# arnavdantuluri/StableTriton

Hardware: AMD Instinct MI355X
Metric: denoise it/s, SDXL UNet 1024x1024 50-step, bs=1 per GPU (higher is better)
Workload: dtype bf16; 1 GPU; SDXL-base UNet, latent 128x128 (1024x1024 px), bs=1/GPU, 50-step Euler-discrete loop, hipGraph mode=step, no CFG; parallelism=prompt-parallel x1, weights=synthetic seed 0, weight_broadcasts=0

## Files before the change

stabletriton_amd/csrc/dispatch.h:

```cpp
#pragma once
#include "gemm_reg.h"
#include "gemm_dma.h"
#include "gemm8p.h"
#ifdef ST_DEV_CONFIGS
#include "../../tools/dev_kernels/gemm4w.h"
void gemm4w_bf16(const GemmArgs& a, hipStream_t st);
void gemm4w_f16(const GemmArgs& a, hipStream_t st);
void gemm4w_fp8(const GemmArgs& a, hipStream_t st);
template <typename T> static inline void gemm4w_call(const GemmArgs& a, hipStream_t st) {
    if constexpr (std::is_same<T, bf16>::value) gemm4w_bf16(a, st);
    else if constexpr (std::is_same<T, f16>::value) gemm4w_f16(a, st);
    else gemm4w_fp8(a, st);
}
#endif

static inline bool colstats_ok(const GemmArgs& a, int bm, bool lnf) {
    const bool ok = a.col_stats && !lnf && (a.N & 3) == 0 && a.rows_per_batch > 0 && a.rows_per_batch % bm == 0 &&
                    cdiv(a.M, bm) <= a.col_tiles_cap;
    if (a.col_rows_out) *a.col_rows_out = ok ? bm : 0;
    return ok;
}

template <typename T, int BM, int BN, int WGM, int WGN, int STAGES, int U, bool CONV, bool GEGLU, bool LNF, bool XA = false>
static void launch_dma_one(const GemmArgs& a, hipStream_t st, int tiles_n) {
    const size_t lds = (size_t)STAGES * U * (BM + BN) * 128 + (size_t)BM * 8 + 1024;
    const int sk = a.splitk > 1 ? a.splitk : 1;
    auto kfn = gemm_dma_kernel<T, BM, BN, WGM, WGN, STAGES, U, CONV, GEGLU, LNF, XA>;
    const bool emit_cols = colstats_ok(a, BM, LNF);
    static unsigned long long lds_ok = 0;
    ensure_dynamic_lds(kfn, lds, &lds_ok);
    GemmArgs b = a;
    {
        static const int force_pm = dev_env_int("ST_GEMM_PANELS", 0);
        const int tiles_m = cdiv(a.M, BM);
        const double abytes = CONV ? (double)a.M * a.Cin * (a.ups ? 0.25 : 1.0) * a.stride * a.stride : (double)a.M * a.K;
        const double wbytes = (double)(GEGLU ? 2 : 1) * a.N * a.K;
        int best_p = 1;
        double best = 1e300;
        for (int pm = 1; pm <= 8; pm *= 2) {
            if (pm > tiles_m) break;
            const double c = abytes * (8.0 / pm) + wbytes * pm;
            if (c < best) { best = c; best_p = pm; }
        }
        if (force_pm > 0) best_p = force_pm > tiles_m ? tiles_m : force_pm;
        b.panel_h = cdiv(tiles_m, best_p);
    }
    const int main_blocks = cdiv(a.M, BM) * tiles_n * sk;
    b.splitk = sk;
    fill_tile_map(b, cdiv(a.M, BM), tiles_n, a.K / ((128 / (int)sizeof(T)) * U));
    static const bool no_helpers = dev_env_int("ST_NO_HELPER_BLOCKS", 0) != 0;
    b.helper_blocks = (b.next_w && main_blocks <= 208 && !no_helpers) ? (256 - main_blocks > 96 ? 96 : 256 - main_blocks) : 0;
    if (!emit_cols) b.col_stats = nullptr;
    fill_next_per(b, main_blocks + b.helper_blocks);
    hipLaunchKernelGGL(kfn, dim3(main_blocks + b.helper_blocks), dim3(WGM * WGN * 64), lds, st, b);
}

template <typename T, int BM, int BN, int WGM, int WGN, int STAGES, int U, bool CONV>
static void launch_dma(const GemmArgs& a, hipStream_t st) {
    if constexpr (!CONV) {
        const bool geglu = a.epi & ST_EPI_GEGLU;
        constexpr bool PAIRS = (BN % 32 == 0);
        if (a.ln_c) {
            if constexpr (PAIRS) {
                if (geglu) { launch_dma_one<T, BM, BN, WGM, WGN, STAGES, U, false, true, true>(a, st, cdiv(a.N, BN / 2)); return; }
            }
            launch_dma_one<T, BM, BN, WGM, WGN, STAGES, U, false, false, true>(a, st, cdiv(a.N, BN));
            return;
        }
        if constexpr (PAIRS) {
            if (geglu) { launch_dma_one<T, BM, BN, WGM, WGN, STAGES, U, false, true, false>(a, st, cdiv(a.N, BN / 2)); return; }
        }
    }
    launch_dma_one<T, BM, BN, WGM, WGN, STAGES, U, CONV, false, false>(a, st, cdiv(a.N, BN));
}

enum { CFG_64x64_S4 = 0, CFG_64x64_S8 = 1, CFG_64x64_S4_U2 = 2, CFG_128x64_S4 = 3, CFG_128x64_S3_U2 = 4,
       CFG_128x128_S3 = 5, CFG_64x64_S3 = 6, CFG_64x64_W8 = 7, CFG_128x64_W8 = 8, CFG_128x128_W8 = 9,
       CFG_64x128_W8 = 10, CFG_64x128_W8_S6 = 11, CFG_128x64_W8_S6 = 12, CFG_128x128_W8_S4 = 13, CFG_64x64_W8_S8 = 14, CFG_64x128_W8_U2 = 15, CFG_128x64_W8_U2 = 16, CFG_64x64_W8_U2 = 17, CFG_256x256_W8 = 18, CFG_256x128_W8 = 19, CFG_128x128_W8_S2 = 20, CFG_128x64_W8_S3 = 21, CFG_64x128_W8_S3 = 22, CFG_128x320_W8 = 23, CFG_128x256_W8 = 24, CFG_64x320_W8 = 25, CFG_64x80_W4 = 26, CFG_128x80_W8 = 27, CFG_128x160_W8 = 28, CFG_128x128_N4_S2 = 29, CFG_128x64_N4_S3 = 30, CFG_64x128_N4_S3 = 31, CFG_256x160_W8_S2 = 32, CFG_COUNT, CFG_256x256_8P = 100, CFG_256x160_8P = 101, CFG_256x256_4W = 102 };

static inline int cfg_bn(int cfg) {
    switch (cfg) {
        case CFG_64x64_S4: case CFG_64x64_S8: case CFG_64x64_S4_U2: case CFG_128x64_S4: case CFG_128x64_S3_U2: case CFG_64x64_S3:
        case CFG_64x64_W8: case CFG_128x64_W8: case CFG_128x64_W8_S6: case CFG_64x64_W8_S8: case CFG_128x64_W8_U2:
        case CFG_64x64_W8_U2: case CFG_128x64_W8_S3: case CFG_128x64_N4_S3: return 64;
        case CFG_256x256_W8: case CFG_128x256_W8: return 256;
        case CFG_128x320_W8: case CFG_64x320_W8: return 320;
        case CFG_64x80_W4: case CFG_128x80_W8: return 80;
        case CFG_128x160_W8: case CFG_256x160_W8_S2: return 160;
        default: return 128;
    }
}

#ifdef ST_DEV_CONFIGS
extern int g_dbg_cfg, g_dbg_fusek;
#endif
static inline int forced_cfg() {
    static int v = dev_env_int("ST_GEMM_FORCE", -1);
#ifdef ST_DEV_CONFIGS
    if (g_dbg_cfg >= 0) return g_dbg_cfg;
#endif
    return v;
}

#ifndef ST_TW_128x128
#define ST_TW_128x128 1.0
#endif
#ifndef ST_TW_64x128
#define ST_TW_64x128 1.0
#endif
#ifndef ST_TW_128x64
#define ST_TW_128x64 1.0
#endif
#ifndef ST_TW_64x64
#define ST_TW_64x64 1.0
#endif
#ifndef ST_TW_128x80
#define ST_TW_128x80 1.0
#endif
#ifndef ST_TW_128x160
#define ST_TW_128x160 1.0
#endif
#ifndef ST_TW_SPLITK
#define ST_TW_SPLITK 1.0
#endif
#ifndef ST_TW_8P
#define ST_TW_8P 1.1
#endif
static inline double model_tweak(int cfg) {
    switch (cfg) {
        case 9: return ST_TW_128x128;
        case 10: return ST_TW_64x128;
        case 8: return ST_TW_128x64;
        case 7: return ST_TW_64x64;
        case 27: return ST_TW_128x80;
        case 28: return ST_TW_128x160;
        default: return 1.0;
    }
}
#ifndef ST_SPLIT_DENSE_TRIP
#define ST_SPLIT_DENSE_TRIP 1.0
#endif
#ifndef ST_SPLIT_160_TRIP
#define ST_SPLIT_160_TRIP 0.8
#endif
// ... 207 lines not shown
```

stabletriton_amd/csrc/epilogue.h:

```cpp
#pragma once
#include "gemm_args.h"

template <typename T, bool GEGLU>
__device__ __forceinline__ void epilogue_compute4(const GemmArgs& p, int m, int n, float (&v)[4], const float (&g_in)[4],
                                                  float ln_mean = 0.f, float ln_rstd = 0.f) {
    const T* __restrict__ bias = (const T*)p.bias;
    const T* __restrict__ Rp = (const T*)p.residual;
    const T* __restrict__ RBp = (const T*)p.rowbias;
    const bool full = (n + 3 < p.N);
    float g[4];
#pragma unroll
    for (int e = 0; e < 4; ++e) g[e] = g_in[e];
    if (p.col_scale) {
        const float rs = p.row_scale[(size_t)m * p.rs_stride];
        for (int e = 0; e < 4 && n + e < p.N; ++e) { v[e] *= rs * p.col_scale[n + e]; if (GEGLU) g[e] *= rs * p.col_scale[p.Ng + n + e]; }
    }
    if (p.ln_c) {
        if (full) {
            float c4[4], d4[4];
            Out4<float>::load(p.ln_c + n, c4); Out4<float>::load(p.ln_d + n, d4);
#pragma unroll
            for (int e = 0; e < 4; ++e) v[e] = ln_fold(v[e], ln_mean, ln_rstd, c4[e], d4[e]);
            if (GEGLU) {
                Out4<float>::load(p.ln_c + p.Ng + n, c4); Out4<float>::load(p.ln_d + p.Ng + n, d4);
// ... 549 lines not shown
    }
    if (has_q8) publish_amax(p.q8_amax, q8_max, blockIdx.x * (NT / 64) + (threadIdx.x >> 6));
    retire_touches(touch_next);
}

template <typename TO, int BM, int BN, int WGM, int WGN, int TM, int TN, bool GEGLU, int LDS_BYTES, bool STATS, bool SCALED = false, typename ColMap>
__device__ __forceinline__ void staged_epilogue(const GemmArgs& p, f32x4 (&acc)[TM][TN], int m0, int n0, int tile_n, int wm, int r16, int q,
                                                ColMap colmap, char* lds, const float2* lnrows) {
    constexpr int VEC = EpiVec<TO>::N;
    constexpr int BNO = GEGLU ? BN / 2 : BN;
    const bool has_res = p.epi & ST_EPI_RESIDUAL, has_rb = p.epi & ST_EPI_ROWBIAS;
    const bool aligned = (m0 + BM <= p.M) && (n0 + BNO <= p.N) && (p.N % VEC == 0) &&
                         (p.C == nullptr || ((p.ldc % VEC == 0) && ((uintptr_t)p.C & 15) == 0)) &&
                         (!has_res || ((p.ldr % VEC == 0) && ((uintptr_t)p.residual & 15) == 0)) && (!has_rb || ((uintptr_t)p.rowbias & 15) == 0) &&
                         ((((uintptr_t)p.bias | (uintptr_t)p.ln_c | (uintptr_t)p.ln_d | (uintptr_t)p.col_scale) & 15) == 0) &&
                         (p.q8_out == nullptr || VEC == 8);
    if (aligned) {
        const int flags = ((p.epi & ST_EPI_BIAS) ? EPI_F_BIAS : 0) | (has_res ? EPI_F_RES : 0) | (has_rb ? EPI_F_RB : 0) | (p.ln_c ? EPI_F_LN : 0) |
                          ((p.epi & ST_EPI_SILU) ? EPI_F_SILU : 0) | (p.col_scale ? EPI_F_SCALE : 0) | ((STATS && p.row_stats) ? EPI_F_ROWS : 0) |
                          ((STATS && p.col_stats && (p.N & 3) == 0) ? EPI_F_COLS : 0) | (p.q8_out ? EPI_F_Q8 : 0) | (p.C ? 0 : EPI_F_NOC) |
                          (p.sp_out ? EPI_F_SP : 0);
#define ST_EPI_CASE(M)                                                                                                                          \
    case (M):                                                                                                                                   \
        staged_epilogue_impl<TO, BM, BN, WGM, WGN, TM, TN, GEGLU, LDS_BYTES, STATS, (M)>(p, acc, m0, n0, tile_n, wm, r16, q, colmap, lds, lnrows); \
        return;
        if constexpr (std::is_same<TO, float>::value) {
            if constexpr (!STATS && !SCALED) {
                switch (flags) { ST_EPI_CASE(EPI_F_LN | EPI_F_SP) default: break; }
            } else if constexpr (STATS && !SCALED) {
                switch (flags) {
                    ST_EPI_CASE(EPI_F_BIAS | EPI_F_ROWS | EPI_F_SP)
                    ST_EPI_CASE(EPI_F_BIAS | EPI_F_RES | EPI_F_ROWS | EPI_F_SP)
                    default: break;
                }
            }
        }
        if constexpr (!STATS && !SCALED) {
            switch (flags) { ST_EPI_CASE(EPI_F_LN) ST_EPI_CASE(EPI_F_LN | EPI_F_BIAS) default: break; }
        } else if constexpr (!STATS && SCALED) {
            switch (flags) {
                ST_EPI_CASE(EPI_F_LN | EPI_F_SCALE)
                ST_EPI_CASE(EPI_F_LN | EPI_F_SCALE | EPI_F_Q8 | EPI_F_NOC)
                default: break;
            }
        } else if constexpr (STATS && !SCALED) {
            switch (flags) {
                ST_EPI_CASE(EPI_F_BIAS)
                ST_EPI_CASE(EPI_F_BIAS | EPI_F_RES)
                ST_EPI_CASE(EPI_F_BIAS | EPI_F_ROWS)
                ST_EPI_CASE(EPI_F_BIAS | EPI_F_RES | EPI_F_ROWS)
                ST_EPI_CASE(EPI_F_BIAS | EPI_F_RES | EPI_F_ROWS | EPI_F_Q8)
                ST_EPI_CASE(EPI_F_BIAS | EPI_F_COLS)
                ST_EPI_CASE(EPI_F_BIAS | EPI_F_RB | EPI_F_COLS)
                ST_EPI_CASE(EPI_F_BIAS | EPI_F_RES | EPI_F_COLS)
                default: break;
            }
        } else {
            switch (flags) {
                ST_EPI_CASE(EPI_F_BIAS | EPI_F_SCALE | EPI_F_RES | EPI_F_ROWS)
                ST_EPI_CASE(EPI_F_BIAS | EPI_F_SCALE | EPI_F_RES | EPI_F_ROWS | EPI_F_Q8)
                default: break;
            }
        }
#undef ST_EPI_CASE
    }
    staged_epilogue_impl<TO, BM, BN, WGM, WGN, TM, TN, GEGLU, LDS_BYTES, STATS, -1>(p, acc, m0, n0, tile_n, wm, r16, q, colmap, lds, lnrows);
}

typedef __attribute__((address_space(3))) void epi_lds_void_t;
typedef __attribute__((address_space(1))) const void epi_gbl_cvoid_t;
__device__ __forceinline__ void touch_next_weights_dma(const GemmArgs& p, unsigned lds_dump_addr) {
    if (!p.next_w || p.helper_blocks > 0) return;
    const size_t lines = p.next_bytes >> 7;
    const size_t per = p.next_per ? (size_t)p.next_per : (lines + gridDim.x - 1) / gridDim.x;
    const size_t lo = (size_t)blockIdx.x * per, hi = lo + per < lines ? lo + per : lines;
    const size_t step = blockDim.x;
    for (size_t l = lo + threadIdx.x; l < hi; l += step)
        __builtin_amdgcn_global_load_lds((epi_gbl_cvoid_t*)((const char*)p.next_w + (touch_line(p, l) << 7)), (epi_lds_void_t*)(uintptr_t)lds_dump_addr, 4, 0, 0);
}

struct DirectCol { int col; bool gate; };
template <int TN, bool GEGLU>
__host__ __device__ __forceinline__ constexpr DirectCol direct_col(int j, int rho) {
    static_assert(TN == 4 || TN == 5, "direct epilogue: wave tiles of 64 or 80 columns");
    const int pc = 8 * (rho >> 2) + (rho & 3);
    if (TN == 4) {
        if (GEGLU) return DirectCol{pc + 4 * (j & 1), j >= 2};
        return DirectCol{32 * (j >> 1) + pc + 4 * (j & 1), false};
    }
    if (GEGLU) {
        if (j < 2) return DirectCol{pc + 4 * j, false};
        if (j > 2) return DirectCol{pc + 4 * (j - 3), true};
        return DirectCol{32 + (rho & 7), rho >= 8};
    }
    if (j < 2) return DirectCol{pc + 4 * j, false};
    if (j > 2) return DirectCol{48 + pc + 4 * (j - 3), false};
    return DirectCol{32 + rho, false};
}
__host__ __device__ __forceinline__ constexpr bool direct_mode_ok(int flags, bool lnf, bool tall) {
    if (lnf) return flags == EPI_F_LN || flags == (EPI_F_LN | EPI_F_BIAS);
    if (flags == 0 || flags == EPI_F_BIAS || flags == (EPI_F_BIAS | EPI_F_RES)) return true;
    return !tall && (flags == (EPI_F_BIAS | EPI_F_ROWS) || flags == (EPI_F_BIAS | EPI_F_RES | EPI_F_ROWS));
}

template <typename TO, int TM, int TN, int WTM, int WTN, int WGM, int WGN, bool GEGLU, int MODE>
__device__ __forceinline__ void direct_epilogue_impl(const GemmArgs& p, f32x4 (&acc)[TM][TN], int m0, int n0, int tile_n, int wm, int wn, int r16, int q,
                                                     char* lds, const float2* lnrows, unsigned lds_dump_addr) {
    static_assert(sizeof(TO) == 2, "direct epilogue: 16-bit outputs");
    constexpr bool has_ln = bool(MODE & EPI_F_LN), has_bias = bool(MODE & EPI_F_BIAS), has_res = bool(MODE & EPI_F_RES), emit_rows = bool(MODE & EPI_F_ROWS);
    typedef typename EpiVec<TO>::type OV;
    typedef typename Raw4<TO>::type R4;
    constexpr int WTNO = GEGLU ? WTN / 2 : WTN;
    constexpr int NW_ = GEGLU ? 1 : 2;
    constexpr bool NARROW = (TN == 5);
    const int nw0 = n0 + wn * WTNO;
    const int lane = (int)(threadIdx.x & 63);
    auto jv_of = [](int w) { return TN == 4 ? 2 * w : (w == 0 ? 0 : 3); };
    auto cb_of = [](int w) { return TN == 4 ? 32 * w : (w == 0 ? 0 : 48); };
    constexpr int JG = TN == 4 ? 2 : 3;
    const bool nlive = !GEGLU || q < 2;
    const int nn = nw0 + 32 + 4 * (GEGLU ? (q & 1) : q);
    const TO* __restrict__ bias = (const TO*)p.bias;

    OV bv[NW_] = {}, bg[NW_] = {};
    f32x4 cv[NW_][2] = {}, dv[NW_][2] = {}, cg[NW_][2] = {}, dg[NW_][2] = {};
    R4 nbv = {}, nbg = {};
    f32x4 ncv = {}, ndv = {}, ncg = {}, ndg = {};
#pragma unroll
    for (int w = 0; w < NW_; ++w) {
        const int n = nw0 + cb_of(w) + 8 * q;
        if (has_bias) { bv[w] = *reinterpret_cast<const OV*>(bias + n); if (GEGLU) bg[w] = *reinterpret_cast<const OV*>(bias + p.Ng + n); }
        if (has_ln) {
#pragma unroll
            for (int h = 0; h < 2; ++h) {
                cv[w][h] = *reinterpret_cast<const f32x4*>(p.ln_c + n + 4 * h); dv[w][h] = *reinterpret_cast<const f32x4*>(p.ln_d + n + 4 * h);
                if (GEGLU) { cg[w][h] = *reinterpret_cast<const f32x4*>(p.ln_c + p.Ng + n + 4 * h); dg[w][h] = *reinterpret_cast<const f32x4*>(p.ln_d + p.Ng + n + 4 * h); }
            }
        }
    }
    if constexpr (NARROW) {
        if (has_bias) { nbv = ld_raw4<TO>(bias + nn); if (GEGLU) nbg = ld_raw4<TO>(bias + p.Ng + nn); }
        if (has_ln) {
            ncv = *reinterpret_cast<const f32x4*>(p.ln_c + nn); ndv = *reinterpret_cast<const f32x4*>(p.ln_d + nn);
            if (GEGLU) { ncg = *reinterpret_cast<const f32x4*>(p.ln_c + p.Ng + nn); ndg = *reinterpret_cast<const f32x4*>(p.ln_d + p.Ng + nn); }
        }
    }
    constexpr int RB_ = (has_res && TM >= 8) ? TM / 2 : TM;
    OV res[has_res ? RB_ : 1][NW_] = {};
    R4 nres[has_res && NARROW ? RB_ : 1] = {};
    auto load_res = [&](int i0) {
        const TO* __restrict__ R = (const TO*)p.residual;
#pragma unroll
        for (int i = 0; i < RB_; ++i) {
            const size_t m = (size_t)(m0 + wm * WTM + (i0 + i) * 16 + r16);
#pragma unroll
            for (int w = 0; w < NW_; ++w) res[has_res ? i : 0][w] = *reinterpret_cast<const OV*>(R + m * p.ldr + nw0 + cb_of(w) + 8 * q);
            if constexpr (NARROW) nres[has_res ? i : 0] = ld_raw4<TO>(R + m * p.ldr + nn);
        }
    };
    if constexpr (has_res) load_res(0);
    float mean[has_ln ? TM : 1] = {}, rstd[has_ln ? TM : 1] = {};
    if constexpr (has_ln) {
#pragma unroll
        for (int i = 0; i < TM; ++i) { const float2 s = lnrows[wm * WTM + i * 16 + r16]; mean[i] = s.x; rstd[i] = s.y; }
    }
    touch_next_weights_dma(p, lds_dump_addr);

    OV outw[TM][NW_];
    R4 outn[NARROW ? TM : 1];
    float rs1[emit_rows ? TM : 1] = {}, rs2[emit_rows ? TM : 1] = {};
#pragma unroll
    for (int i = 0; i < TM; ++i) {
        if constexpr (has_res && RB_ < TM) { if (i == RB_) { __builtin_amdgcn_sched_barrier(0); load_res(RB_); } }
#pragma unroll
        for (int w = 0; w < NW_; ++w) {
            const int jv = jv_of(w);
#pragma unroll
            for (int e = 0; e < 8; ++e) {
                float v = acc[i][jv + (e >> 2)][e & 3];
                float g = GEGLU ? acc[i][JG + (e >> 2)][e & 3] : 0.f;
                if (has_ln) { v = ln_fold(v, mean[i], rstd[i], cv[w][e >> 2][e & 3], dv[w][e >> 2][e & 3]); if (GEGLU) g = ln_fold(g, mean[i], rstd[i], cg[w][e >> 2][e & 3], dg[w][e >> 2][e & 3]); }
                if (has_bias) { v += Elem<TO>::to_f(bv[w][e]); if (GEGLU) g += Elem<TO>::to_f(bg[w][e]); }
                if (GEGLU) v *= gelu_for<TO>(g);
                if (has_res) v += Elem<TO>::to_f(res[has_res ? i % RB_ : 0][w][e]);
                const TO o = Elem<TO>::from_f(v);
                outw[i][w][e] = o;
                if (emit_rows) { const float s = Elem<TO>::to_f(o); rs1[i] += s; rs2[i] = fmaf(s, s, rs2[i]); }
            }
        }
        if constexpr (NARROW) {
#pragma unroll
            for (int e = 0; e < 4; ++e) {
                float v = acc[i][2][e];
                float g = 0.f;
                if (GEGLU) g = __shfl(v, (lane + 32) & 63, 64);
                if (has_ln) { v = ln_fold(v, mean[i], rstd[i], ncv[e], ndv[e]); if (GEGLU) g = ln_fold(g, mean[i], rstd[i], ncg[e], ndg[e]); }
                if (has_bias) { v += Elem<TO>::to_f(nbv[e]); if (GEGLU) g += Elem<TO>::to_f(nbg[e]); }
                if (GEGLU) v *= gelu_for<TO>(g);
                if (has_res) v += Elem<TO>::to_f(nres[has_res ? i % RB_ : 0][e]);
                const TO o = Elem<TO>::from_f(v);
                outn[i][e] = o;
                if (emit_rows && nlive) { const float s = Elem<TO>::to_f(o); rs1[i] += s; rs2[i] = fmaf(s, s, rs2[i]); }
            }
        }
        if constexpr (emit_rows) __builtin_amdgcn_sched_barrier(0);
    }
    TO* __restrict__ C = (TO*)p.C;
#pragma unroll
    for (int i = 0; i < TM; ++i) {
        const size_t m = (size_t)(m0 + wm * WTM + i * 16 + r16);
#pragma unroll
        for (int w = 0; w < NW_; ++w) *reinterpret_cast<OV*>(C + m * p.ldc + nw0 + cb_of(w) + 8 * q) = outw[i][w];
        if constexpr (NARROW) { if (nlive) *reinterpret_cast<R4*>(C + m * p.ldc + nn) = outn[i]; }
    }
    if constexpr (emit_rows) {
        float2* sm = reinterpret_cast<float2*>(lds);
#pragma unroll
        for (int i = 0; i < TM; ++i) {
            float a1 = rs1[i], a2 = rs2[i];
            a1 += __shfl_xor(a1, 16, 64); a2 += __shfl_xor(a2, 16, 64);
            a1 += __shfl_xor(a1, 32, 64); a2 += __shfl_xor(a2, 32, 64);
            if (q == 0) sm[(wm * WTM + i * 16 + r16) * WGN + wn] = make_float2(a1, a2);
        }
        __syncthreads();
        for (int row = threadIdx.x; row < WGM * WTM; row += WGM * WGN * 64) {
            float a1 = 0.f, a2 = 0.f;
#pragma unroll
            for (int w = 0; w < WGN; ++w) { const float2 x = sm[row * WGN + w]; a1 += x.x; a2 += x.y; }
            reinterpret_cast<float2*>(p.row_stats)[(size_t)(m0 + row) * p.stats_chunks + tile_n] = make_float2(a1, a2);
        }
    }
    asm volatile("s_waitcnt vmcnt(0)" ::: "memory");
}

static __host__ __device__ __forceinline__ int direct_flags(const GemmArgs& p, bool lnf, bool tall) {
    if ((p.epi & (ST_EPI_ROWBIAS | ST_EPI_SILU)) || p.col_scale || p.q8_out || p.sp_out || !p.C || (!lnf && p.col_stats) || (lnf && p.row_stats)) return -1;
    const int f = ((p.epi & ST_EPI_BIAS) ? EPI_F_BIAS : 0) | ((p.epi & ST_EPI_RESIDUAL) ? EPI_F_RES : 0) | (p.ln_c ? EPI_F_LN : 0) | (p.row_stats ? EPI_F_ROWS : 0);
    return direct_mode_ok(f, lnf, tall) ? f : -1;
}

template <typename TO, int TM, int TN, int WTM, int WTN, int WGM, int WGN, bool GEGLU, bool LNF>
__device__ __forceinline__ void direct_epilogue(const GemmArgs& p, f32x4 (&acc)[TM][TN], int m0, int n0, int tile_n, int wm, int wn, int r16, int q,
                                                char* lds, const float2* lnrows, unsigned lds_dump_addr) {
    const int flags = direct_flags(p, LNF, TM >= 8);
#define ST_DIR_CASE(M)                                                                                                        \
    case (M):                                                                                                                 \
        direct_epilogue_impl<TO, TM, TN, WTM, WTN, WGM, WGN, GEGLU, (M)>(p, acc, m0, n0, tile_n, wm, wn, r16, q, lds, lnrows, lds_dump_addr); \
        return;
    if constexpr (LNF) {
        switch (flags) { ST_DIR_CASE(EPI_F_LN) ST_DIR_CASE(EPI_F_LN | EPI_F_BIAS) default: break; }
    } else {
        switch (flags) { ST_DIR_CASE(0) ST_DIR_CASE(EPI_F_BIAS) ST_DIR_CASE(EPI_F_BIAS | EPI_F_RES) default: break; }
        if constexpr (TM < 8) {
            switch (flags) { ST_DIR_CASE(EPI_F_BIAS | EPI_F_ROWS) ST_DIR_CASE(EPI_F_BIAS | EPI_F_RES | EPI_F_ROWS) default: break; }
        }
    }
#undef ST_DIR_CASE
}
```

stabletriton_amd/csrc/gemm_dma.h:

```cpp
#pragma once
#include "epilogue.h"

static __device__ __attribute__((aligned(16))) unsigned int g_zero16[4] = {0u, 0u, 0u, 0u};

typedef __attribute__((address_space(3))) void lds_void_t;
typedef __attribute__((address_space(1))) const void gbl_cvoid_t;

template <int AUX = 0>
__device__ __forceinline__ void dma16(const void* src, char* lds_wave_base) {
    __builtin_amdgcn_global_load_lds((gbl_cvoid_t*)src, (lds_void_t*)lds_wave_base, 16, 0, AUX);
}

constexpr int dma_before_last_group(int G, int NG) {
    int n = 0;
    for (int e = 0; e < G; ++e) n += (e * NG / G < NG - 1) ? 1 : 0;
    return n;
}

constexpr int dma_in_group(int G, int NG, int g) {
    int n = 0;
    for (int e = 0; e < G; ++e) n += (e * NG / G == g) ? 1 : 0;
    return n;
}

// ... 11 lines not shown
template <int TPR>
struct LnRowSum {
    static_assert(TPR == 1 || TPR == 2 || TPR == 4 || TPR == 8, "threads per row");
    static constexpr int RES = 8 / TPR;
    static constexpr int PRE = 8 / RES;
    float2 pre[RES][PRE];
    __device__ __forceinline__ void load(const float2* row, int chunks, int part) {
#pragma unroll
        for (int j = 0; j < RES; ++j)
#pragma unroll
            for (int i = 0; i < PRE; ++i) {
                const int c = part + TPR * j + 8 * i;
                pre[j][i] = row[c < chunks ? c : 0];
            }
    }
    __device__ __forceinline__ void finish(const float2* row, int chunks, int part, float& s1, float& s2) {
        float a1[RES], a2[RES];
#pragma unroll
        for (int j = 0; j < RES; ++j) {
            a1[j] = 0.f; a2[j] = 0.f;
#pragma unroll
            for (int i = 0; i < PRE; ++i) {
                const bool ok = part + TPR * j + 8 * i < chunks;
                a1[j] += ok ? pre[j][i].x : 0.f; a2[j] += ok ? pre[j][i].y : 0.f;
            }
            for (int c = part + TPR * j + 8 * PRE; c < chunks; c += 8) { const float2 v = row[c]; a1[j] += v.x; a2[j] += v.y; }
#pragma unroll
            for (int o = 1; o < TPR; o <<= 1) { a1[j] += __shfl_xor(a1[j], o, 64); a2[j] += __shfl_xor(a2[j], o, 64); }
        }
#pragma unroll
        for (int w = 1; w < RES; w <<= 1)
#pragma unroll
            for (int j = 0; j + w < RES; j += 2 * w) { a1[j] += a1[j + w]; a2[j] += a2[j + w]; }
        s1 = a1[0]; s2 = a2[0];
    }
};

template <int TM, int TN, int TILE_ELEMS>
__device__ __forceinline__ bool splitk_combine(const GemmArgs& p, f32x4 (&acc)[TM][TN], int tw, int split, char* lds, int t, int wave, int lane) {
    float* slab0 = p.partial + (size_t)tw * p.splitk * TILE_ELEMS;
    {
        asm volatile("s_nop 7\n\ts_nop 7\n\ts_nop 2" ::: "memory");
        float* mine = slab0 + (size_t)split * TILE_ELEMS + (size_t)wave * (TM * TN * 256) + lane * 4;
#pragma unroll
        for (int i = 0; i < TM; ++i)
#pragma unroll
            for (int j = 0; j < TN; ++j) {
                const float* dst = mine + (i * TN + j) * 256;
                asm volatile("global_store_dwordx4 %0, %1, off sc1\n\ts_nop 1" ::"v"(dst), "v"(acc[i][j]) : "memory");
            }
    }
    asm volatile("s_waitcnt vmcnt(0)" ::: "memory");
    __syncthreads();
    int* flag = reinterpret_cast<int*>(lds);
    if (t == 0) *flag = __hip_atomic_fetch_add(p.tile_counters + tw, 1, __ATOMIC_RELAXED, __HIP_MEMORY_SCOPE_AGENT);
    __syncthreads();
    if (*flag != p.splitk - 1) return false;
    if (t == 0) __hip_atomic_store(p.tile_counters + tw, 0, __ATOMIC_RELAXED, __HIP_MEMORY_SCOPE_AGENT);
    f32x4 own[TM][TN];
#pragma unroll
    for (int i = 0; i < TM; ++i)
#pragma unroll
        for (int j = 0; j < TN; ++j) { own[i][j] = acc[i][j]; acc[i][j] = (f32x4){0.f, 0.f, 0.f, 0.f}; }
    typedef unsigned int u32x4_ __attribute__((ext_vector_type(4)));
    const __amdgpu_buffer_rsrc_t slabs = __builtin_amdgcn_make_buffer_rsrc((void*)slab0, 0, (int)((size_t)p.splitk * TILE_ELEMS * 4), 0x00020000);
    for (int sl = 0; sl < p.splitk; ++sl) {
        if (sl == split) {
#pragma unroll
            for (int i = 0; i < TM; ++i)
#pragma unroll
                for (int j = 0; j < TN; ++j) acc[i][j] += own[i][j];
            continue;
        }
        const int off = (sl * TILE_ELEMS + wave * (TM * TN * 256) + lane * 4) * 4;
#pragma unroll
        for (int i = 0; i < TM; ++i)
#pragma unroll
            for (int j = 0; j < TN; ++j)
                acc[i][j] += __builtin_bit_cast(f32x4, (u32x4_)__builtin_amdgcn_raw_buffer_load_b128(slabs, off + (i * TN + j) * 1024, 0, 16));
    }
    return true;
}

template <typename T, int BM, int BN, int WGM, int WGN, int STAGES, int U, bool CONV, bool GEGLU, bool LNF = false, bool XA = false>
__global__ __launch_bounds__(WGM* WGN * 64) void gemm_dma_kernel(const GemmArgs p) {
    constexpr int NW = WGM * WGN;
    constexpr int VEC = 16 / (int)sizeof(T);
    constexpr int KB = 8 * VEC;
    constexpr int WTM = BM / WGM, WTN = BN / WGN;
    constexpr int TM = WTM / 16, TN = WTN / 16;
    constexpr int A_PIECES = BM / 8, B_PIECES = BN / 8;
    constexpr int A_IT = (A_PIECES + NW - 1) / NW, B_IT = (B_PIECES + NW - 1) / NW;
    constexpr bool UNEVEN = (A_PIECES % NW != 0) || (B_PIECES % NW != 0);
    constexpr int G = (A_IT + B_IT) * U;
    constexpr int A_BYTES = BM * 128, TILE = (BM + BN) * 128, STAGE = TILE * U;
    static_assert(!GEGLU || (BN % 32 == 0), "GEGLU: value and gate halves of the tile are whole 16-column accumulator tiles");
    static_assert((STAGES - 2) * G <= 63, "vmcnt immediate");
    typedef typename Mma<T>::Frag Frag;
    typedef typename OutT<T>::type TO;

    extern __shared__ __attribute__((aligned(16))) char lds[];
    char* const dump = lds + STAGES * STAGE + BM * 8;

    const int t = threadIdx.x, lane = t & 63;
    const int wave = __builtin_amdgcn_readfirstlane(t >> 6);
    const int wm = wave / WGN, wn = wave - wm * WGN;
    const int tiles_m = (p.M + BM - 1) / BM;
    const int nblk = gridDim.x - p.helper_blocks, bid = blockIdx.x;
    if (bid >= nblk) {
        unsigned int sink = 0;
        touch_next_weights(p, sink, true);
        retire_touches(sink);
        return;
    }
    constexpr int BNO = GEGLU ? BN / 2 : BN;
    const TileId tid = tile_of_block(p, bid, nblk);
    const int split = tid.split, tw = tid.tw, tile_m = tid.tile_m, tile_n = tid.tile_n;
    const int m0 = tile_m * BM;
    const int n0 = tile_n * BNO;

    const T* __restrict__ Ap = (const T*)p.A;
    const T* __restrict__ Wp = (const T*)p.W;
    const T* zeros = reinterpret_cast<const T*>(g_zero16);

    const int lr = lane >> 3;
    const int lc = (lane & 7) ^ lr;
    const T* a_ptr[A_IT];
    const T* a2_ptr[CONV ? A_IT : 1];
    int a_adv[A_IT], a_iy[A_IT], a_ix[A_IT];
#pragma unroll
    for (int i = 0; i < A_IT; ++i) {
        const int row = (wave + i * NW) * 8 + lr;
        const int m = m0 + row;
        const bool ok = m < p.M && (!UNEVEN || wave + i * NW < A_PIECES);
        if (CONV && p.A2) {
            a_ptr[i] = Ap + (size_t)(ok ? m : 0) * p.Csplit + lc * VEC;
            a2_ptr[i] = (const T*)p.A2 + (size_t)(ok ? m : 0) * (p.Cin - p.Csplit) + lc * VEC;
            a_iy[i] = ok ? 0 : -(1 << 28); a_ix[i] = 0; a_adv[i] = 0;
        } else if (CONV) {
            const int hw = p.Hout * p.Wout;
            const int mm = ok ? m : 0;
            const int img = mm / hw, rem = mm - img * hw;
            const int oy = rem / p.Wout, ox = rem - oy * p.Wout;
            a_iy[i] = ok ? oy * p.stride - p.pad : -(1 << 28);
            a_ix[i] = ox * p.stride - p.pad;
            a_ptr[i] = Ap + (size_t)img * p.Hin * p.Win * p.Cin + lc * VEC;
            a_adv[i] = 0;
        } else {
            a_ptr[i] = ok ? Ap + (size_t)m * p.lda + lc * VEC : zeros;
            a_adv[i] = ok ? KB : 0;
            a_iy[i] = a_ix[i] = 0;
        }
    }
    const T* b_ptr[B_IT];
    int b_adv[B_IT];
#pragma unroll
    for (int i = 0; i < B_IT; ++i) {
        const int row = (wave + i * NW) * 8 + lr;
        int wrow;
        bool ok;
        if (GEGLU) {
            const int half = row >= BN / 2 ? 1 : 0;
            const int ncol = n0 + row - half * (BN / 2);
            ok = ncol < p.N && (!UNEVEN || wave + i * NW < B_PIECES);
            wrow = ncol + half * p.Ng;
        } else {
            wrow = n0 + row;
            ok = wrow < p.N && (!UNEVEN || wave + i * NW < B_PIECES);
        }
        b_ptr[i] = ok ? Wp + (size_t)wrow * p.K + lc * VEC : zeros;
        b_adv[i] = ok ? KB : 0;
    }

    unsigned int touch_sink = 0;
    {
        constexpr int NT_ = NW * 64;
        const int ncols_out = min(BNO, p.N - n0);
        auto touch_at = [&](const char* a) {
            a = (const char*)((uintptr_t)a & ~(uintptr_t)3);
            asm volatile("global_load_dword %0, %1, off" : "+v"(touch_sink) : "v"(a) : "memory");
        };
        auto touch = [&](const void* base, long byte_off, int nbytes) {
            for (int o = t * 128; o < nbytes; o += NT_ * 128) touch_at((const char*)base + byte_off + o);
        };
        if (p.epi & ST_EPI_BIAS) {
            touch(p.bias, (long)n0 * sizeof(TO), ncols_out * (int)sizeof(TO));
            if (GEGLU) touch(p.bias, ((long)p.Ng + n0) * sizeof(TO), ncols_out * (int)sizeof(TO));
        }
        if (LNF) {
            touch(p.ln_c, (long)n0 * 4, ncols_out * 4); touch(p.ln_d, (long)n0 * 4, ncols_out * 4);
            if (GEGLU) { touch(p.ln_c, ((long)p.Ng + n0) * 4, ncols_out * 4); touch(p.ln_d, ((long)p.Ng + n0) * 4, ncols_out * 4); }
        }
        if (p.epi & ST_EPI_RESIDUAL) {
            const int lines = (ncols_out * (int)sizeof(TO) + 127) / 128;
            const int rows = min(BM, p.M - m0);
            for (int o = t; o < rows * lines; o += NT_) {
                const int r = o / lines, l = o - r * lines;
                touch_at((const char*)p.residual + ((size_t)(m0 + r) * p.ldr + n0) * sizeof(TO) + l * 128);
            }
        }
    }

    const int nk_lo = split * p.nk_base + min(split, p.nk_rem), nk_hi = nk_lo + p.nk_base + (split < p.nk_rem ? 1 : 0);
    const int kbase = nk_lo * U;
    constexpr int PER_TILE = A_IT + B_IT;
    int cs_r = 0, cs_s = 0, cs_c0 = 0;
    if (CONV) {
        if (p.korder) {
            const int taps = p.R_ * p.S;
            const int cs = kbase / taps, tap = kbase - cs * taps;
            cs_c0 = cs * KB; cs_r = tap / p.S; cs_s = tap - cs_r * p.S;
        } else {
            const int k0 = kbase * KB;
            const int tap = k0 / p.Cin;
            cs_c0 = k0 - tap * p.Cin; cs_r = tap / p.S; cs_s = tap - cs_r * p.S;
        }
    }
    auto conv_advance = [&](bool go) {
        if (p.korder) {
            cs_s += go ? 1 : 0;
            const bool w1 = cs_s == p.S;
            cs_s = w1 ? 0 : cs_s;
            cs_r += w1 ? 1 : 0;
            const bool w2 = cs_r == p.R_;
            cs_r = w2 ? 0 : cs_r;
            cs_c0 += w2 ? KB : 0;
        } else {
            cs_c0 += go ? KB * U : 0;
            const bool w1 = cs_c0 >= p.Cin;
            cs_c0 -= w1 ? p.Cin : 0;
            cs_s += w1 ? 1 : 0;
            const bool w2 = cs_s == p.S;
            cs_s = w2 ? 0 : cs_s;
            cs_r += w2 ? 1 : 0;
        }
    };
    const unsigned lds_base = lds_addr_of(lds), dump_addr = lds_base + STAGES * STAGE + BM * 8;
    auto issue_one = [&](int st, int buf, int e) {
        const int u = e / PER_TILE, i = e - u * PER_TILE;
        const int kt = kbase + st * U + u;
        const unsigned base = lds_base + buf * STAGE + u * TILE;
        if (i < A_IT) {
            const T* src;
            if (CONV) {
                int r, s_, c0;
                if constexpr (U == 1) {
                    r = cs_r; s_ = cs_s; c0 = cs_c0;
                } else {
                    const int k0 = kt * KB;
                    const int tap = k0 / p.Cin;
                    c0 = k0 - tap * p.Cin; r = tap / p.S; s_ = tap - r * p.S;
                }
                int iy = a_iy[i] + r, ix = a_ix[i] + s_;
                bool ok;
                if (p.ups) {
                    ok = iy >= 0 && ix >= 0 && iy < 2 * p.Hin && ix < 2 * p.Win;
                    iy >>= 1; ix >>= 1;
                } else {
// ... 78 lines not shown
            const int c = 4 * (g & 1) + q;
            return *reinterpret_cast<const Frag*>(base + row * 128 + ((c ^ (row & 7)) << 4));
        }
    };
    auto read_group = [&](int buf, int g, int set) {
        const char* sa = lds + buf * STAGE + (g / GPT) * TILE;
        const char* sb = sa + A_BYTES;
#pragma unroll
        for (int i = 0; i < TM; ++i) fa[set][i] = read_frag(sa, wm * WTM + i * 16 + r16, g);
#pragma unroll
        for (int j = 0; j < TN; ++j) fb[set][j] = read_frag(sb, wn * WTN + j * 16 + r16, g);
    };
    auto mma_group = [&](int set) {
#pragma unroll
        for (int i = 0; i < TM; ++i)
#pragma unroll
            for (int j = 0; j < TN; ++j) {
                if constexpr (is_split<T>()) Mma<T>::run2(acc[i][j], corr[i][j], fb[set][j], fa[set][i]);
                else Mma<T>::run(acc[i][j], fb[set][j], fa[set][i]);
            }
    };

    int cur = 0, nxt = STAGES - 1;
    read_group(0, 0, 0);
    auto trip = [&](int kt, auto par_) {
        constexpr int PAR = decltype(par_)::value;
        const int pf = min(kt + STAGES - 1, nk - 1);
        auto group = [&](auto gc) {
            constexpr int g = decltype(gc)::value;
            if constexpr (g + 1 < NG) {
                read_group(cur, g + 1, (g + 1 + PAR) & 1);
            } else {
                wait_vmcnt<EARLY ? 0 : (STAGES - 3) * G + dma_before_last_group(G, NG)>();
                __builtin_amdgcn_s_barrier();
                __builtin_amdgcn_sched_barrier(0);
                read_group(cur + 1 == STAGES ? 0 : cur + 1, 0, (g + 1 + PAR) & 1);
            }
            constexpr int n_dma = EARLY ? (g == 0 ? G : 0) : dma_in_group(G, NG, g);
#pragma unroll
            for (int e = 0; e < G; ++e)
                if ((EARLY ? 0 : e * NG / G) == g) issue_one(pf, nxt, e);
            mma_group((g + PAR) & 1);
            __builtin_amdgcn_sched_group_barrier(0x100, (TM + TN) * RPF, 0);
            if constexpr (n_dma > 0) __builtin_amdgcn_sched_group_barrier(0x020, n_dma, 0);
            __builtin_amdgcn_sched_group_barrier(0x008, TM * TN * mfma_per_frag<T>(), 0);
            __builtin_amdgcn_sched_barrier(0);
        };
        group(std::integral_constant<int, 0>{});
        if constexpr (NG > 1) group(std::integral_constant<int, 1>{});
        if constexpr (NG > 2) {
            group(std::integral_constant<int, 2>{});
            group(std::integral_constant<int, 3>{});
        }
        __builtin_amdgcn_s_waitcnt(0xc07f);
        cur = cur + 1 == STAGES ? 0 : cur + 1;
        nxt = nxt + 1 == STAGES ? 0 : nxt + 1;
        if (CONV) conv_advance(kt + STAGES - 1 < nk - 1);
    };
    if constexpr (NG % 2 == 0) {
        for (int kt = 0; kt < nk; ++kt) trip(kt, std::integral_constant<int, 0>{});
    } else {
        for (int kt = 0; kt < nk; kt += 2) {
            trip(kt, std::integral_constant<int, 0>{});
            if (kt + 1 < nk) trip(kt + 1, std::integral_constant<int, 1>{});
        }
    }
    wait_vmcnt<0>();
    if constexpr (is_split<T>()) {
#pragma unroll
        for (int i = 0; i < TM; ++i)
#pragma unroll
            for (int j = 0; j < TN; ++j)
#pragma unroll
                for (int e = 0; e < 4; ++e) acc[i][j][e] = __builtin_fmaf(corr[i][j][e], ST_SPLIT_INV, acc[i][j][e]);
    }
    if (p.splitk > 1) {
        if (!splitk_combine<TM, TN, BM * BN>(p, acc, tw, split, lds, t, wave, lane)) {
            unsigned int sink = 0;
            touch_next_weights(p, sink);
            retire_touches(sink);
            return;
        }
    }
    if constexpr (XA) {
        static_assert(LNF && !GEGLU && !CONV && BM == 128 && BN == 64 && NW == 8 && sizeof(T) == 2, "xattn epilogue: 128 x 64 tile, 8 waves, 16-bit elements");
        static_assert(STAGES * STAGE >= 16384 + 3 * 16384, "xattn epilogue: Q tile + K/V ring fit the GEMM's ring");
        const float2* lnst = reinterpret_cast<const float2*>(lds + STAGES * STAGE);
        float mean[TM], rstd[TM];
#pragma unroll
        for (int i = 0; i < TM; ++i) {
            const float2 v = lnst[wm * WTM + i * 16 + r16];
            mean[i] = v.x; rstd[i] = v.y;
        }
        __syncthreads();
        T* qt = reinterpret_cast<T*>(lds);
#pragma unroll
        for (int j = 0; j < TN; ++j) {
            const int col = wn * WTN + j * 16 + 4 * q;
            const f32x4 cv = *reinterpret_cast<const f32x4*>(p.ln_c + n0 + col), dv = *reinterpret_cast<const f32x4*>(p.ln_d + n0 + col);
#pragma unroll
            for (int i = 0; i < TM; ++i) {
                const int row = wm * WTM + i * 16 + r16;
                typename V16<T>::x4 o4;
#pragma unroll
                for (int e = 0; e < 4; ++e) o4[e] = (T)ln_fold(acc[i][j][e], mean[i], rstd[i], cv[e], dv[e]);
                *reinterpret_cast<typename V16<T>::x4*>(qt + row * 64 + col) = o4;
            }
        }
        __syncthreads();
        const int bimg = m0 / p.xa_T, head = tile_n;
        const T* Kb = (const T*)p.xa_k + (size_t)bimg * p.xa_S * p.xa_ldk + (size_t)head * 64;
        const T* Vb = (const T*)p.xa_v + (size_t)bimg * p.xa_S * p.xa_ldv + (size_t)head * 64;
        attn16_core<T, 8>(qt, 64, 128, Kb, Vb, p.xa_ldk, p.xa_ldv, p.xa_S, (T*)p.C + (size_t)m0 * p.ldc + (size_t)head * 64, p.ldc,
                       min(BM, p.M - m0), p.xa_scale_log2e, lds + 16384, wave, lane);
        unsigned int sink = 0;
        touch_next_weights(p, sink);
        retire_touches(sink);
    } else if constexpr (BM * BN >= 128 * 128 || GEGLU || CONV) {
        staged_epilogue<TO, BM, BN, WGM, WGN, TM, TN, GEGLU, STAGES * STAGE, !LNF, is_fp8<T>()>(
            p, acc, m0, n0, tile_n, wm, r16, q, ColsPlain{wn, WTN}, lds, reinterpret_cast<const float2*>(lds + STAGES * STAGE));
    } else if constexpr (LNF) {
        float mean[TM], rstd[TM];
        const float2* lnst = reinterpret_cast<const float2*>(lds + STAGES * STAGE);
#pragma unroll
        for (int i = 0; i < TM; ++i) {
            const float2 v = lnst[wm * WTM + i * 16 + r16];
            mean[i] = v.x; rstd[i] = v.y;
        }
        const bool inside = (m0 + BM <= p.M) && (n0 + BNO <= p.N) && (p.N & 3) == 0 && p.C != nullptr && !p.q8_out && !p.sp_out;
        const int flags = inside ? (((p.epi & ST_EPI_BIAS) ? EPI_F_BIAS : 0) | (p.epi & (ST_EPI_RESIDUAL | ST_EPI_ROWBIAS | ST_EPI_SILU) ? 1024 : 0) |
                                    (p.col_scale ? EPI_F_SCALE : 0) | EPI_F_LN) : -1;
        if (!is_fp8<T>() && flags == EPI_F_LN) gemm_epilogue<TO, TM, TN, WTM, WTN, GEGLU, 0, 0, false, EPI_F_LN>(p, acc, m0, n0, wm, wn, r16, q, split, mean, rstd);
        else if (!is_fp8<T>() && flags == (EPI_F_LN | EPI_F_BIAS))
            gemm_epilogue<TO, TM, TN, WTM, WTN, GEGLU, 0, 0, false, EPI_F_LN | EPI_F_BIAS>(p, acc, m0, n0, wm, wn, r16, q, split, mean, rstd);
        else if (is_fp8<T>() && flags == (EPI_F_LN | EPI_F_SCALE))
            gemm_epilogue<TO, TM, TN, WTM, WTN, GEGLU, 0, 0, false, EPI_F_LN | EPI_F_SCALE>(p, acc, m0, n0, wm, wn, r16, q, split, mean, rstd);
        else gemm_epilogue<TO, TM, TN, WTM, WTN, GEGLU>(p, acc, m0, n0, wm, wn, r16, q, split, mean, rstd);
    } else {
        const bool inside = (m0 + BM <= p.M) && (n0 + BNO <= p.N) && (p.N & 3) == 0 && p.C != nullptr;
        const int flags = inside ? (((p.epi & ST_EPI_BIAS) ? EPI_F_BIAS : 0) | ((p.epi & ST_EPI_RESIDUAL) ? EPI_F_RES : 0) | ((p.epi & ST_EPI_ROWBIAS) ? EPI_F_RB : 0) |
                                    ((p.epi & ST_EPI_SILU) ? EPI_F_SILU : 0) | (p.col_scale ? EPI_F_SCALE : 0) | (p.ln_c ? EPI_F_LN : 0) | (p.row_stats ? EPI_F_ROWS : 0) |
                                    ((p.col_stats && (p.N & 3) == 0) ? EPI_F_COLS : 0) | (p.q8_out ? EPI_F_Q8 : 0) | (p.sp_out ? EPI_F_SP : 0)) : -1;
#define ST_FRAG_CASE(M)                                                                                                                        \
    case (M):                                                                                                                                  \
        gemm_epilogue<TO, TM, TN, WTM, WTN, GEGLU, WGM, WGN, false, (M)>(p, acc, m0, n0, wm, wn, r16, q, split, nullptr, nullptr, lds, tile_n); \
        break;
        bool done = false;
        if constexpr (std::is_same<TO, float>::value) {
            done = true;
            switch (flags) {
                ST_FRAG_CASE(EPI_F_BIAS | EPI_F_ROWS | EPI_F_SP)
                ST_FRAG_CASE(EPI_F_BIAS | EPI_F_RES | EPI_F_ROWS | EPI_F_SP)
                default: done = false;
            }
        }
        if (done) {
        } else if constexpr (!is_fp8<T>()) {
            switch (flags) {
                ST_FRAG_CASE(EPI_F_BIAS)
                ST_FRAG_CASE(EPI_F_BIAS | EPI_F_RES)
                ST_FRAG_CASE(EPI_F_BIAS | EPI_F_ROWS)
                ST_FRAG_CASE(EPI_F_BIAS | EPI_F_RES | EPI_F_ROWS)
                ST_FRAG_CASE(EPI_F_BIAS | EPI_F_RES | EPI_F_ROWS | EPI_F_Q8)
                ST_FRAG_CASE(EPI_F_BIAS | EPI_F_RES | EPI_F_COLS)
                default: gemm_epilogue<TO, TM, TN, WTM, WTN, GEGLU, WGM, WGN>(p, acc, m0, n0, wm, wn, r16, q, split, nullptr, nullptr, lds, tile_n);
            }
        } else {
// ... 10 lines not shown
```

Measured before the change: 77.11 it/s.

## Add direct register epilogue for 128x64 LDS-DMA GEMM tiles with permuted weight rows

```diff
diff --git a/stabletriton_amd/csrc/dispatch.h b/stabletriton_amd/csrc/dispatch.h
--- a/stabletriton_amd/csrc/dispatch.h
+++ b/stabletriton_amd/csrc/dispatch.h
@@ -21,11 +21,21 @@
     return ok;
 }
 
-template <typename T, int BM, int BN, int WGM, int WGN, int STAGES, int U, bool CONV, bool GEGLU, bool LNF, bool XA = false>
+template <typename T>
+static inline bool dma_direct(const GemmArgs& a, int bm, int bn) {
+    if constexpr (sizeof(T) != 2) return false;
+    static const bool off = dev_env_int("ST_DMA_DIRECT", 1) == 0;
+    if (off || (a.epi & ST_EPI_GEGLU) || direct_flags(a, a.ln_c != nullptr, false) < 0) return false;
+    if (a.M % bm != 0 || a.N % bn != 0) return false;
+    auto al16 = [](const void* p_) { return ((uintptr_t)p_ & 15) == 0; };
+    return a.ldc % 8 == 0 && al16(a.C) && (!(a.epi & ST_EPI_RESIDUAL) || (a.ldr % 8 == 0 && al16(a.residual))) && al16(a.bias) && al16(a.ln_c) && al16(a.ln_d);
+}
+
+template <typename T, int BM, int BN, int WGM, int WGN, int STAGES, int U, bool CONV, bool GEGLU, bool LNF, bool XA = false, bool DIRECT = false>
 static void launch_dma_one(const GemmArgs& a, hipStream_t st, int tiles_n) {
     const size_t lds = (size_t)STAGES * U * (BM + BN) * 128 + (size_t)BM * 8 + 1024;
     const int sk = a.splitk > 1 ? a.splitk : 1;
-    auto kfn = gemm_dma_kernel<T, BM, BN, WGM, WGN, STAGES, U, CONV, GEGLU, LNF, XA>;
+    auto kfn = gemm_dma_kernel<T, BM, BN, WGM, WGN, STAGES, U, CONV, GEGLU, LNF, XA, DIRECT>;
     const bool emit_cols = colstats_ok(a, BM, LNF);
     static unsigned long long lds_ok = 0;
     ensure_dynamic_lds(kfn, lds, &lds_ok);
@@ -60,6 +70,14 @@
     if constexpr (!CONV) {
         const bool geglu = a.epi & ST_EPI_GEGLU;
         constexpr bool PAIRS = (BN % 32 == 0);
+        constexpr bool CAN_DIRECT = sizeof(T) == 2 && BM == 128 && BN == 64 && WGM == 4 && WGN == 2 && STAGES == 4 && U == 1;
+        if constexpr (CAN_DIRECT) {
+            if (dma_direct<T>(a, BM, BN)) {
+                if (a.ln_c) launch_dma_one<T, BM, BN, WGM, WGN, STAGES, U, false, false, true, false, true>(a, st, a.N / BN);
+                else launch_dma_one<T, BM, BN, WGM, WGN, STAGES, U, false, false, false, false, true>(a, st, a.N / BN);
+                return;
+            }
+        }
         if (a.ln_c) {
             if constexpr (PAIRS) {
                 if (geglu) { launch_dma_one<T, BM, BN, WGM, WGN, STAGES, U, false, true, true>(a, st, cdiv(a.N, BN / 2)); return; }
diff --git a/stabletriton_amd/csrc/epilogue.h b/stabletriton_amd/csrc/epilogue.h
--- a/stabletriton_amd/csrc/epilogue.h
+++ b/stabletriton_amd/csrc/epilogue.h
@@ -655,8 +655,10 @@
 struct DirectCol { int col; bool gate; };
 template <int TN, bool GEGLU>
 __host__ __device__ __forceinline__ constexpr DirectCol direct_col(int j, int rho) {
-    static_assert(TN == 4 || TN == 5, "direct epilogue: wave tiles of 64 or 80 columns");
+    static_assert(TN == 2 || TN == 4 || TN == 5, "direct epilogue: wave tiles of 32, 64 or 80 columns");
+    static_assert(TN != 2 || !GEGLU, "direct epilogue: the 32-column wave tiles carry no GEGLU");
     const int pc = 8 * (rho >> 2) + (rho & 3);
+    if (TN == 2) return DirectCol{pc + 4 * j, false};
     if (TN == 4) {
         if (GEGLU) return DirectCol{pc + 4 * (j & 1), j >= 2};
         return DirectCol{32 * (j >> 1) + pc + 4 * (j & 1), false};
@@ -676,15 +678,36 @@
     return !tall && (flags == (EPI_F_BIAS | EPI_F_ROWS) || flags == (EPI_F_BIAS | EPI_F_RES | EPI_F_ROWS));
 }
 
-template <typename TO, int TM, int TN, int WTM, int WTN, int WGM, int WGN, bool GEGLU, int MODE>
+template <typename TO, int TM>
+struct DirectPre {
+    typename EpiVec<TO>::type bv;
+    f32x4 cv[2], dv[2];
+    typename EpiVec<TO>::type res[TM];
+};
+template <typename TO, int TM, bool LNF>
+__device__ __forceinline__ void direct_preload(const GemmArgs& p, DirectPre<TO, TM>& pre, int m_first, int n) {
+    typedef typename EpiVec<TO>::type OV;
+    if (p.epi & ST_EPI_BIAS) pre.bv = *reinterpret_cast<const OV*>((const TO*)p.bias + n);
+    if constexpr (LNF) {
+#pragma unroll
+        for (int h = 0; h < 2; ++h) { pre.cv[h] = *reinterpret_cast<const f32x4*>(p.ln_c + n + 4 * h); pre.dv[h] = *reinterpret_cast<const f32x4*>(p.ln_d + n + 4 * h); }
+    }
+    if (p.epi & ST_EPI_RESIDUAL) {
+#pragma unroll
+        for (int i = 0; i < TM; ++i) pre.res[i] = *reinterpret_cast<const OV*>((const TO*)p.residual + (size_t)(m_first + i * 16) * p.ldr + n);
+    }
+}
+
+template <typename TO, int TM, int TN, int WTM, int WTN, int WGM, int WGN, bool GEGLU, int MODE, int ORDER = 0>
 __device__ __forceinline__ void direct_epilogue_impl(const GemmArgs& p, f32x4 (&acc)[TM][TN], int m0, int n0, int tile_n, int wm, int wn, int r16, int q,
-                                                     char* lds, const float2* lnrows, unsigned lds_dump_addr) {
+                                                     char* lds, const float2* lnrows, unsigned lds_dump_addr, const DirectPre<TO, TM>* pre = nullptr) {
     static_assert(sizeof(TO) == 2, "direct epilogue: 16-bit outputs");
+    static_assert(ORDER == 0 || (ORDER == 1 && TN == 2), "direct epilogue: the fragment order of the statistics is rebuilt for the 32-column wave tiles");
     constexpr bool has_ln = bool(MODE & EPI_F_LN), has_bias = bool(MODE & EPI_F_BIAS), has_res = bool(MODE & EPI_F_RES), emit_rows = bool(MODE & EPI_F_ROWS);
     typedef typename EpiVec<TO>::type OV;
     typedef typename Raw4<TO>::type R4;
     constexpr int WTNO = GEGLU ? WTN / 2 : WTN;
-    constexpr int NW_ = GEGLU ? 1 : 2;
+    constexpr int NW_ = (GEGLU || TN == 2) ? 1 : 2;
     constexpr bool NARROW = (TN == 5);
     const int nw0 = n0 + wn * WTNO;
     const int lane = (int)(threadIdx.x & 63);
@@ -694,6 +717,7 @@
     const bool nlive = !GEGLU || q < 2;
     const int nn = nw0 + 32 + 4 * (GEGLU ? (q & 1) : q);
     const TO* __restrict__ bias = (const TO*)p.bias;
+    if constexpr (emit_rows && ORDER != 0) __builtin_amdgcn_s_barrier();
 
     OV bv[NW_] = {}, bg[NW_] = {};
     f32x4 cv[NW_][2] = {}, dv[NW_][2] = {}, cg[NW_][2] = {}, dg[NW_][2] = {};
@@ -702,6 +726,11 @@
 #pragma unroll
     for (int w = 0; w < NW_; ++w) {
         const int n = nw0 + cb_of(w) + 8 * q;
+        if (pre) {
+            if (has_bias) bv[w] = pre->bv;
+            if (has_ln) { cv[w][0] = pre->cv[0]; cv[w][1] = pre->cv[1]; dv[w][0] = pre->dv[0]; dv[w][1] = pre->dv[1]; }
+            continue;
+        }
         if (has_bias) { bv[w] = *reinterpret_cast<const OV*>(bias + n); if (GEGLU) bg[w] = *reinterpret_cast<const OV*>(bias + p.Ng + n); }
         if (has_ln) {
 #pragma unroll
@@ -725,6 +754,7 @@
         const TO* __restrict__ R = (const TO*)p.residual;
 #pragma unroll
         for (int i = 0; i < RB_; ++i) {
+            if (pre) { res[has_res ? i : 0][0] = pre->res[i0 + i]; continue; }
             const size_t m = (size_t)(m0 + wm * WTM + (i0 + i) * 16 + r16);
 #pragma unroll
             for (int w = 0; w < NW_; ++w) res[has_res ? i : 0][w] = *reinterpret_cast<const OV*>(R + m * p.ldr + nw0 + cb_of(w) + 8 * q);
@@ -758,8 +788,22 @@
                 if (has_res) v += Elem<TO>::to_f(res[has_res ? i % RB_ : 0][w][e]);
                 const TO o = Elem<TO>::from_f(v);
                 outw[i][w][e] = o;
-                if (emit_rows) { const float s = Elem<TO>::to_f(o); rs1[i] += s; rs2[i] = fmaf(s, s, rs2[i]); }
-            }
+                if (emit_rows && ORDER != 1) { const float s = Elem<TO>::to_f(o); rs1[i] += s; rs2[i] = fmaf(s, s, rs2[i]); }
+            }
+        }
+        if constexpr (emit_rows && ORDER == 1) {
+            float h1[2], h2[2];
+#pragma unroll
+            for (int h = 0; h < 2; ++h) {
+                float a1 = 0.f, a2 = 0.f;
+#pragma unroll
+                for (int e = 0; e < 4; ++e) { const float s = Elem<TO>::to_f(outw[i][0][4 * h + e]); a1 += s; a2 = fmaf(s, s, a2); }
+                a1 = __shfl_xor(a1, 32, 64); a2 = __shfl_xor(a2, 32, 64);
+#pragma unroll
+                for (int e = 0; e < 4; ++e) { const float s = Elem<TO>::to_f(outw[i][0][4 * h + e]); a1 += s; a2 = fmaf(s, s, a2); }
+                h1[h] = a1; h2[h] = a2;
+            }
+            rs1[i] = h1[0] + h1[1]; rs2[i] = h2[0] + h2[1];
         }
         if constexpr (NARROW) {
 #pragma unroll
@@ -792,10 +836,15 @@
         for (int i = 0; i < TM; ++i) {
             float a1 = rs1[i], a2 = rs2[i];
             a1 += __shfl_xor(a1, 16, 64); a2 += __shfl_xor(a2, 16, 64);
-            a1 += __shfl_xor(a1, 32, 64); a2 += __shfl_xor(a2, 32, 64);
-            if (q == 0) sm[(wm * WTM + i * 16 + r16) * WGN + wn] = make_float2(a1, a2);
-        }
-        __syncthreads();
+            if constexpr (ORDER == 0) { a1 += __shfl_xor(a1, 32, 64); a2 += __shfl_xor(a2, 32, 64); }
+            if (q == (ORDER == 1 ? 2 : 0)) sm[(wm * WTM + i * 16 + r16) * WGN + wn] = make_float2(a1, a2);
+        }
+        if constexpr (ORDER == 0) {
+            __syncthreads();
+        } else {
+            asm volatile("s_waitcnt lgkmcnt(0)" ::: "memory");
+            __builtin_amdgcn_s_barrier();
+        }
         for (int row = threadIdx.x; row < WGM * WTM; row += WGM * WGN * 64) {
             float a1 = 0.f, a2 = 0.f;
 #pragma unroll
@@ -830,3 +879,24 @@
     }
 #undef ST_DIR_CASE
 }
+
+template <typename TO, int TM, int TN, int WTM, int WTN, int WGM, int WGN, bool LNF, int ORDER>
+__device__ __forceinline__ void direct_epilogue_dma(const GemmArgs& p, f32x4 (&acc)[TM][TN], int m0, int n0, int tile_n, int wm, int wn, int r16, int q,
+                                                    char* lds, const float2* lnrows, unsigned lds_dump_addr, const DirectPre<TO, TM>& pre) {
+    static_assert(TM < 8 && TN == 2, "direct epilogue of the LDS-DMA tiles: 32-column wave tiles, not tall");
+    const int flags = direct_flags(p, LNF, false);
+#define ST_DIR_CASE(M)                                                                                                               \
+    case (M):                                                                                                                        \
+        direct_epilogue_impl<TO, TM, TN, WTM, WTN, WGM, WGN, false, (M), ORDER>(p, acc, m0, n0, tile_n, wm, wn, r16, q, lds, lnrows, lds_dump_addr, &pre); \
+        return;
+    if constexpr (LNF) {
+        switch (flags) { ST_DIR_CASE(EPI_F_LN) ST_DIR_CASE(EPI_F_LN | EPI_F_BIAS) default: break; }
+    } else {
+        switch (flags) {
+            ST_DIR_CASE(0) ST_DIR_CASE(EPI_F_BIAS) ST_DIR_CASE(EPI_F_BIAS | EPI_F_RES)
+            ST_DIR_CASE(EPI_F_BIAS | EPI_F_ROWS) ST_DIR_CASE(EPI_F_BIAS | EPI_F_RES | EPI_F_ROWS)
+            default: break;
+        }
+    }
+#undef ST_DIR_CASE
+}
diff --git a/stabletriton_amd/csrc/gemm_dma.h b/stabletriton_amd/csrc/gemm_dma.h
--- a/stabletriton_amd/csrc/gemm_dma.h
+++ b/stabletriton_amd/csrc/gemm_dma.h
@@ -117,7 +117,7 @@
     return true;
 }
 
-template <typename T, int BM, int BN, int WGM, int WGN, int STAGES, int U, bool CONV, bool GEGLU, bool LNF = false, bool XA = false>
+template <typename T, int BM, int BN, int WGM, int WGN, int STAGES, int U, bool CONV, bool GEGLU, bool LNF = false, bool XA = false, bool DIRECT = false>
 __global__ __launch_bounds__(WGM* WGN * 64) void gemm_dma_kernel(const GemmArgs p) {
     constexpr int NW = WGM * WGN;
     constexpr int VEC = 16 / (int)sizeof(T);
@@ -131,6 +131,7 @@
     constexpr int A_BYTES = BM * 128, TILE = (BM + BN) * 128, STAGE = TILE * U;
     static_assert(!GEGLU || (BN % 32 == 0), "GEGLU: value and gate halves of the tile are whole 16-column accumulator tiles");
     static_assert((STAGES - 2) * G <= 63, "vmcnt immediate");
+    static_assert(!DIRECT || (!CONV && !GEGLU && !XA && sizeof(T) == 2 && TN == 2 && TM < 8 && !UNEVEN), "direct epilogue: dense 16-bit tiles of 32-column wave tiles");
     typedef typename Mma<T>::Frag Frag;
     typedef typename OutT<T>::type TO;
 
@@ -199,6 +200,10 @@
             const int ncol = n0 + row - half * (BN / 2);
             ok = ncol < p.N && (!UNEVEN || wave + i * NW < B_PIECES);
             wrow = ncol + half * p.Ng;
+        } else if constexpr (DIRECT) {
+            const int wc = row / WTN, in = row - wc * WTN;
+            wrow = n0 + wc * WTN + direct_col<TN, false>(in >> 4, in & 15).col;
+            ok = wrow < p.N;
         } else {
             wrow = n0 + row;
             ok = wrow < p.N && (!UNEVEN || wave + i * NW < B_PIECES);
@@ -208,7 +213,10 @@
     }
 
     unsigned int touch_sink = 0;
-    {
+    DirectPre<TO, DIRECT ? TM : 1> pre = {};
+    if constexpr (DIRECT) {
+        direct_preload<TO, TM, LNF>(p, pre, m0 + wm * WTM + (lane & 15), n0 + wn * WTN + 8 * (lane >> 4));
+    } else {
         constexpr int NT_ = NW * 64;
         const int ncols_out = min(BNO, p.N - n0);
         auto touch_at = [&](const char* a) {
@@ -453,7 +461,11 @@
             return;
         }
     }
-    if constexpr (XA) {
+    if constexpr (DIRECT) {
+        static_assert(BM * BN < 128 * 128, "direct epilogue: the tiles that finished in the fragment epilogue");
+        direct_epilogue_dma<TO, TM, TN, WTM, WTN, WGM, WGN, LNF, 1>(
+            p, acc, m0, n0, tile_n, wm, wn, r16, q, lds, reinterpret_cast<const float2*>(lds + STAGES * STAGE), dump_addr, pre);
+    } else if constexpr (XA) {
         static_assert(LNF && !GEGLU && !CONV && BM == 128 && BN == 64 && NW == 8 && sizeof(T) == 2, "xattn epilogue: 128 x 64 tile, 8 waves, 16-bit elements");
         static_assert(STAGES * STAGE >= 16384 + 3 * 16384, "xattn epilogue: Q tile + K/V ring fit the GEMM's ring");
         const float2* lnst = reinterpret_cast<const float2*>(lds + STAGES * STAGE);
```

Result: no change. 77.76 it/s, median of 6 (+0.8%).
